# MarSaKi/VLN-BEVBert

Measured on AMD Instinct MI355X. Metric: pretrain_samples_per_sec, higher is better.
Workload: dtype bf16+fp32-residual

## Files before the change

include/bevbert_hip.h:

```cpp
#ifndef BEVBERT_HIP_H
#define BEVBERT_HIP_H

#include <stdint.h>

#ifdef __cplusplus
extern "C" {
#endif

typedef struct ihipStream_t* hipStream_t;

#define BEVBERT_F32 0
#define BEVBERT_BF16 1
#define BEVBERT_F16 2

const char* bevbert_last_error(void);
int bevbert_version(void);
int bevbert_hip_error_reset(void);
const char* bevbert_arch(void);
const char* bevbert_attn_last_path(int backward);
const char* bevbert_attn_plan(int B, int nh, int Lq, int Lk, int dtype, int impl, int has_key_mask, int has_bias,
                              float drop_p, int has_bits, int bits_ready, int want_dbias, int ncu, int backward);

int bevbert_bev_lift_bin(const float* depths, const float* T_c2w, const float* T_w2c, const float* S_w2c,
                         const float* pix_scale, int B, int V, int hw, float depth_scale, int dim, float res,
// ... 25 lines not shown
                                                float drop_p, uint64_t seed, uint64_t offset, hipStream_t stream);
int bevbert_layernorm_post_fwd(const void* x, const float* bias, const float* gamma, const float* beta,
                               const void* post1, const void* post2, void* y, void* z_out, float* mean, float* rstd,
                               int rows, int H, float eps, int dtype, hipStream_t stream);
int bevbert_layernorm_bwd(const void* dy, const void* z, const float* mean, const float* rstd, const float* gamma,
                          void* dz, void* dx, float* dgamma, float* dbeta, float* dbias, float* workspace, int rows,
                          int H, int dtype, float drop_p, uint64_t seed, uint64_t offset, int accumulate,
                          hipStream_t stream);
int bevbert_layernorm_bwd_add(const void* dy, const void* z, const float* mean, const float* rstd, const float* gamma,
                              void* dz, void* dx, const void* dz_add, float* dgamma, float* dbeta, float* dbias,
                              float* workspace, int rows, int H, int dtype, float drop_p, uint64_t seed, uint64_t offset,
                              int accumulate, hipStream_t stream);
int bevbert_layernorm_res32_fwd(const void* x, const float* bias, const void* residual, int residual_dtype,
                                const float* gamma, const float* beta, void* y16, float* y32, float* z32, float* mean,
                                float* rstd, int rows, int H, float eps, float drop_p, uint64_t seed, uint64_t offset,
                                hipStream_t stream);
int bevbert_layernorm_res32_chain_fwd(const void* x, const float* bias, const float* z_prev, const float* mean_prev,
                                      const float* rstd_prev, const float* gamma_prev, const float* beta_prev,
                                      const float* gamma, const float* beta, void* y16, float* y32, float* z32,
                                      float* mean, float* rstd, int rows, int H, float eps, float drop_p, uint64_t seed,
                                      uint64_t offset, hipStream_t stream);
int bevbert_layernorm_res32_bwd(const void* dy16, const float* dy32, const float* z32, const float* mean,
                                const float* rstd, const float* gamma, void* dz, void* dx16, float* dgamma,
                                float* dbeta, float* dbias, float* workspace, int rows, int H, float drop_p, uint64_t seed,
                                uint64_t offset, int accumulate, int dz_dtype,
                                hipStream_t stream);
int64_t bevbert_colsum_workspace_floats(int total_cols);
int bevbert_colsum_partial_rows(int rows);
int bevbert_colsum_finalize(const float* partials, int nblocks, int nwhich, int C, float* out0, float* out1,
                            float* out2, int accumulate, hipStream_t stream);
int bevbert_colsum_partials(const void* dy, float* partials, int rows, int C, int dtype, hipStream_t stream);
int bevbert_multi_finalize(const void* tasks, int ntasks, hipStream_t stream);
int bevbert_multi_accum(const void* tasks, int ntasks, hipStream_t stream);
int bevbert_set_fold_norm_slots(float* slots, int capacity);
int bevbert_sumsq_tasks(const void* tasks, int ntasks, hipStream_t stream);

int bevbert_embed_sum_layernorm_fwd(const int64_t* ids, const void* word, const void* pos, const void* type_row,
                                    const float* gamma, const float* beta, void* y, void* z_out, float* mean,
                                    float* rstd, int rows, int L, int H, float eps, int dtype, float drop_p,
                                    uint64_t seed, uint64_t offset, hipStream_t stream);

int bevbert_embedding_grad(const int64_t* ids, const void* d, float* table_grad, int rows, int H, int padding_idx,
                           int dtype, hipStream_t stream);

int64_t bevbert_smallk_workspace_floats(int rows, int K, int H);
int bevbert_smallk_linear_layernorm_fwd(const float* feat, const float* weight, const float* bias, const float* gamma,
                                        const float* beta, const void* post1, const void* table, const int64_t* idx,
                                        void* y, float* mean, float* rstd, int rows, int K, int H, float eps, int dtype,
                                        hipStream_t stream);
int bevbert_smallk_linear_layernorm_bwd(const void* dy, const float* feat, const float* weight, const float* bias,
                                        const float* mean, const float* rstd, const float* gamma, float* dweight,
                                        float* dbias, float* dgamma, float* dbeta, float* workspace, int rows, int K,
                                        int H, int dtype, hipStream_t stream);

int bevbert_colsum_any(const void* dy, float* out, int rows, int C, int dtype, int accumulate, hipStream_t stream);

int bevbert_weighted_mean_fwd(const float* x, const float* w, const float* denom_dev, float denom, int n, float* out,
                              hipStream_t stream);
int bevbert_weighted_mean_bwd(const float* dout, const float* w, const float* denom_dev, float denom, int n, float* dx,
                              hipStream_t stream);

int bevbert_sem_select(const uint8_t* mask1, const uint8_t* mask2, int n, int cap, int classes, int64_t* idx, float* valid,
                       float* denom, hipStream_t stream);
int bevbert_bce_rows_fwd(const void* logits, const uint8_t* labels, const int64_t* idx, float* out, int rows, int C, int dtype,
                         hipStream_t stream);
int bevbert_bce_rows_bwd(const void* logits, const uint8_t* labels, const int64_t* idx, const float* g, void* dlogits, int rows,
// ... 286 lines not shown
```

vln_bevbert_amd/arena.py:

```python
import math

import torch

from . import lib
from .lib import ptr, stream


def call(name, *args):
    from . import ops
    return ops.call(name, *args)

CHUNK = 1024
_ZERO_KERNEL = __import__("os").environ.get("BEVBERT_ZERO_KERNEL", "0") == "1"
NO_DECAY = ("bias", "LayerNorm.bias", "LayerNorm.weight")


def _round_up(n, m):
    return (n + m - 1) // m * m


class ParamArena:
    _serial = 0

    def __init__(self, module, device, compute_dtype=torch.float32, groups=()):
# ... 40 lines not shown
        self._flags_host = torch.zeros(off // CHUNK, dtype=torch.uint8)
        self._seg_of = {}
        for start, end, decay, seg in seg_meta:
            if decay:
                self._flags_host[start // CHUNK:end // CHUNK] |= 1
            for n in seg:
                self._seg_of[n] = (start // CHUNK, end // CHUNK)
        self.flags = self._flags_host.to(dev)
        self.chunk_steps = torch.zeros(off // CHUNK, dtype=torch.int32, device=dev)
        self._touched = set()
        self._flags_dirty = False
        self.publish_grads = True
        self.allreduce_group = None
        self.defer_allreduce = False
        self._cb_queued = False
        self._fresh = []
        self._published = []
        self._param_versions = None
        self.step_count = 0
        self._scalars = torch.zeros(4, dtype=torch.float32, device=dev)
        self._partials = torch.zeros(1024, dtype=torch.float32, device=dev)
        self.named = named
        for n, p in named:
            o, k = self.slices[n]
            view = self.params[o:o + k].view(p.shape)
            view.copy_(p.data.to(dev, torch.float32))
            p.data = view
            p.main_grad = self.grads[o:o + k].view(p.shape)
            p.compute = self.shadow[o:o + k].view(p.shape) if self.shadow is not None else p.data
            p.arena = self
            p.arena_name = n
        self._index = {n: i for i, (n, _) in enumerate(named)}
        self.fold_store = False
        ParamArena._serial += 1
        self.fold_key = ("arena", ParamArena._serial)
        tables = {id(m.weight) for m in module.modules() if isinstance(m, torch.nn.Embedding)}
        self._fold_ranges = []
        for o, k, _ in sorted((*self.slices[n], n) for n, p in named if p.dim() >= 2 and id(p) not in tables):
            if self._fold_ranges and self._fold_ranges[-1][1] == o:
                self._fold_ranges[-1][1] = o + k
            else:
                self._fold_ranges.append([o, o + k])
        self._fold_starts = [a for a, _ in self._fold_ranges]
        self._fold_comp = {}
        self.sync_shadow()
        self._param_versions = sum(p._version for _, p in named)

    def packed(self, names, shape):
        o0, _ = self.slices[names[0]]
        total = 0
        for n in names:
            o, k = self.slices[n]
            assert o == o0 + total, f"{names} are not contiguous in the arena"
            total += k
        assert total == math.prod(shape)
        src = self.shadow if self.shadow is not None else self.params
        return src[o0:o0 + total].view(shape), self.grads[o0:o0 + total].view(shape)

    def touch(self, param):
        n = param.arena_name
        if n not in self._touched:
            self._touched.add(n)
            a, b = self._seg_of[n]
            self._flags_host[a:b] |= 2
            self._flags_dirty = True
        if self.publish_grads:
# ... 48 lines not shown
        if v != self._param_versions:
            if self._param_versions is not None:
                self.sync_shadow()
            self._param_versions = v

    def sync_shadow(self):
        if self.shadow is not None:
            call("bevbert_cast_f32", ptr(self.params), ptr(self.shadow), self.numel, lib.dtype_code(self.compute_dtype),
                 stream())

    def sync(self):
        if self.device.type == "cuda":
            from . import ops
            ops.WgradStream.flush_all()
            cur = torch.cuda.current_stream(self.device)
            for side in ops.Branches.side_streams():
                if ops.Branches.enabled or side not in ops.WgradStream.streams or ops.WgradStream.dirty:
                    cur.wait_stream(side)
            ops.WgradStream.dirty = False
            ops.WgradStream.release()

    def store_ok(self, sink_ptr, n):
        import bisect
        off, rem = divmod(sink_ptr - self.grads.data_ptr(), 4)
        if rem or off < 0 or off + n > self.numel:
            return False
        i = bisect.bisect_right(self._fold_starts, off) - 1
        return i >= 0 and off + n <= self._fold_ranges[i][1]

    def _arm_fold(self):
        from . import ops
        ops.ReduceQueue.store_ok = self.store_ok if self.fold_store else None
        ops.ReduceQueue.fold_norm = None

    def _name_at(self, sink_ptr):
        off = (sink_ptr - self.grads.data_ptr()) // 4
        return next((n for n, (o, k) in self.slices.items() if o <= off < o + k), f"arena offset {off}")

    def fold_check_zero(self, stores):
        base = self.grads.data_ptr()
        views = [self.grads[(p - base) // 4:(p - base) // 4 + n] for p, n in stores]
        counts = torch.stack([torch.count_nonzero(v) for v in views]).tolist()
        bad = [(self._name_at(p), c) for (p, _), c in zip(stores, counts) if c]
        if bad:
            raise lib.BevBertHipError(
                "store-mode fold: the gradient of " + ", ".join(f"{n} ({c} non-zero elements)" for n, c in bad[:4])
                + " is not zero before the step's fold -- something other than the split-K fold writes it, or the arena "
                "was not zeroed for this step (BEVBERT_FOLD_STORE=0 turns the store mode off)")

    def _fold_complement(self, entry):
        ent = self._fold_comp.get(id(entry))
        if ent is not None and ent[0] is entry:
            return ent[1:]
        if torch.cuda.is_current_stream_capturing():
            raise lib.BevBertHipError("fold-norm complement table missing during graph capture (warm-up steps build it)")
        import numpy as np
        base, recs, pos = self.grads.data_ptr(), [], 0
        for p, n, _ in sorted(entry["norm_jobs"]) + [(base + 4 * self.numel, 0, 0)]:
            o = (p - base) // 4
            for a in range(pos, o, 16384):
                recs.append((base + 4 * a, (min(a + 16384, o) - a) // 4))
            pos = o + n
            assert pos % 4 == 0, "fold sinks are float4-aligned"
        from . import ops
        if entry["nslots"] + len(recs) > ops.ReduceQueue.SLOT_CAPACITY:
            return None
# ... 116 lines not shown
```

vln_bevbert_amd/csrc/optimizer.hip:

```cpp
#include <math.h>
#include <type_traits>

#include "rowops_common.h"

#define ACCUM_U 4
#define ACCUM_SC 4
template <typename T, bool STORE = false>
__device__ __forceinline__ float accum_fold(const T* part_, float* sink_, size_t stride4, size_t n4, int S, size_t first,
                                            size_t step) {
  const BB_GLOBAL T* __restrict__ part = (const BB_GLOBAL T*)part_;
  BB_GLOBAL float* __restrict__ sink = (BB_GLOBAL float*)sink_;
  float sq = 0.f;
  for (size_t i = first; i < n4; i += ACCUM_U * step) {
    size_t idx[ACCUM_U];
    float4 acc[ACCUM_U];
#pragma unroll
    for (int u = 0; u < ACCUM_U; ++u) {
      idx[u] = i + u * step < n4 ? i + u * step : n4 - 1;
      if constexpr (STORE) acc[u] = make_float4(0.f, 0.f, 0.f, 0.f);
      else acc[u] = gld4<float>(sink + idx[u] * 4);
    }
    int s = 0;
    for (; s + ACCUM_SC <= S; s += ACCUM_SC) {
      float4 v[ACCUM_SC][ACCUM_U];
// ... 29 lines not shown
                                                             int S, size_t n4) {
  accum_fold<T>(partials, sink, n4, n4, S, (size_t)blockIdx.x * 256 + threadIdx.x, (size_t)gridDim.x * 256);
}

struct AccumTask {
  const void* partials;
  float* sink;
  unsigned long long n4_total;
  unsigned int off4, n4;
  int S, dtype;
};
#define ACCUM_STORE 0x100
#define ACCUM_NORM 0x200
__device__ __forceinline__ float block_sum_256(float s) {
  __shared__ float sh[4];
  s = wave_sum(s);
  if ((threadIdx.x & 63) == 0) sh[threadIdx.x >> 6] = s;
  __syncthreads();
  return (sh[0] + sh[1]) + (sh[2] + sh[3]);
}
template <typename T, bool STORE>
__device__ __forceinline__ float accum_task(const AccumTask& t) {
  return accum_fold<T, STORE>((const T*)t.partials + (size_t)t.off4 * 4, t.sink, t.n4_total, t.n4, t.S, threadIdx.x, 256);
}
__global__ __launch_bounds__(256) void multi_accum_kernel(const AccumTask* __restrict__ tasks, float* __restrict__ slots,
                                                          unsigned int capacity) {
  const AccumTask t = tasks[blockIdx.x];
  const bool bf16 = (t.dtype & 0xff) == BB_BF16;
  float sq;
  if (t.dtype & ACCUM_STORE) sq = bf16 ? accum_task<bf16_raw, true>(t) : accum_task<float, true>(t);
  else sq = bf16 ? accum_task<bf16_raw, false>(t) : accum_task<float, false>(t);
  const unsigned int slot = (unsigned int)t.dtype >> 12;
  if ((t.dtype & ACCUM_NORM) && slot < capacity) {
    sq = block_sum_256(sq);
    if (threadIdx.x == 0) slots[slot] = sq;
  }
}

__global__ __launch_bounds__(256) void sumsq_kernel(const float* __restrict__ g, size_t n4, float* __restrict__ partials) {
  float s = 0.f;
  for (size_t i = (size_t)blockIdx.x * 256 + threadIdx.x; i < n4; i += (size_t)gridDim.x * 256) {
    const float4 v = *reinterpret_cast<const float4*>(g + i * 4);
    s += (v.x * v.x + v.y * v.y) + (v.z * v.z + v.w * v.w);
  }
  __shared__ float sh[4];
  s = wave_sum(s);
  if ((threadIdx.x & 63) == 0) sh[threadIdx.x >> 6] = s;
  __syncthreads();
  if (threadIdx.x == 0) partials[blockIdx.x] = (sh[0] + sh[1]) + (sh[2] + sh[3]);
}

struct SumsqTask {
  const float* ptr;
  unsigned int n4, slot;
};
__global__ __launch_bounds__(256) void sumsq_tasks_kernel(const SumsqTask* __restrict__ tasks, float* __restrict__ slots,
                                                          unsigned int capacity) {
  const SumsqTask t = tasks[blockIdx.x];
  if (t.slot >= capacity) return;
  const unsigned int n4 = t.n4 < 4096u ? t.n4 : 4096u;
  float s = 0.f;
  if (n4) {
    const BB_GLOBAL float* __restrict__ g = (const BB_GLOBAL float*)t.ptr;
    float4 v[16];
#pragma unroll
    for (int u = 0; u < 16; ++u) {
// ... 76 lines not shown
template <typename TO>
__global__ __launch_bounds__(256) void cast_f32_kernel(const float* __restrict__ src, TO* __restrict__ dst, size_t n4) {
  for (size_t i = (size_t)blockIdx.x * 256 + threadIdx.x; i < n4; i += (size_t)gridDim.x * 256)
    st4<TO>(dst + i * 4, *reinterpret_cast<const float4*>(src + i * 4));
}

BEVBERT_API int bevbert_accum_partials(const void* partials, float* sink, int S, int64_t n, int dtype,
                                       hipStream_t stream) {
  BB_REQUIRE(n % 4 == 0 && S >= 1, "accum_partials: n must be a multiple of 4 and S >= 1");
  if (n == 0) return BB_OK;
  size_t nb = ((size_t)n / 4 + 255) / 256;
  if (nb > 8192) nb = 8192;
  const bool type_ok = bb_with_type(dtype, [&](auto t) {
    using T = decltype(t);
    hipLaunchKernelGGL(accum_partials_kernel<T>, dim3(nb), dim3(256), 0, stream, (const T*)partials, sink, S, (size_t)n / 4);
  });
  if (!type_ok) return bb_dtype_unsupported("accum_partials", dtype);
  BB_CHECK_LAUNCH("accum_partials");
  return BB_OK;
}

BEVBERT_API int bevbert_multi_accum(const void* tasks, int ntasks, hipStream_t stream) {
  static_assert(sizeof(AccumTask) == 40, "AccumTask is part of the C ABI");
  if (ntasks <= 0) return BB_OK;
  BB_REQUIRE(tasks != nullptr, "multi_accum: null task table");
  int capacity = 0;
  float* slots = bb_fold_norm_slots(&capacity);
  hipLaunchKernelGGL(multi_accum_kernel, dim3(ntasks), dim3(256), 0, stream, (const AccumTask*)tasks, slots,
                     (unsigned int)(slots ? capacity : 0));
  BB_CHECK_LAUNCH("multi_accum");
  return BB_OK;
}

BEVBERT_API int bevbert_sumsq_tasks(const void* tasks, int ntasks, hipStream_t stream) {
  static_assert(sizeof(SumsqTask) == 16, "SumsqTask is part of the C ABI");
  if (ntasks <= 0) return BB_OK;
  int capacity = 0;
  float* slots = bb_fold_norm_slots(&capacity);
  BB_REQUIRE(tasks != nullptr && slots != nullptr, "sumsq_tasks: null task table, or no slot array registered");
  hipLaunchKernelGGL(sumsq_tasks_kernel, dim3(ntasks), dim3(256), 0, stream, (const SumsqTask*)tasks, slots,
                     (unsigned int)capacity);
  BB_CHECK_LAUNCH("sumsq_tasks");
  return BB_OK;
}

BEVBERT_API int bevbert_grad_norm_clip(const float* grads, int64_t n, float pre_scale, float max_norm,
                                       float* partials, float* scalars, hipStream_t stream) {
  BB_REQUIRE(n % 4 == 0, "grad_norm_clip: n must be a multiple of 4");
  hipLaunchKernelGGL(sumsq_kernel, dim3(1024), dim3(256), 0, stream, grads, (size_t)n / 4, partials);
  hipLaunchKernelGGL(clip_coef_kernel, dim3(1), dim3(256), 0, stream, partials, 1024, pre_scale, max_norm, scalars);
  BB_CHECK_LAUNCH("grad_norm_clip");
  return BB_OK;
}

BEVBERT_API int bevbert_clip_from_slots(const float* slots, int n, float pre_scale, float max_norm, float* scalars,
                                        hipStream_t stream) {
  BB_REQUIRE(n >= 0 && (slots != nullptr || n == 0) && scalars != nullptr, "clip_from_slots: null pointer or negative count");
  hipLaunchKernelGGL(clip_coef_kernel, dim3(1), dim3(256), 0, stream, slots, n, pre_scale, max_norm, scalars);
  BB_CHECK_LAUNCH("clip_from_slots");
  return BB_OK;
}

BEVBERT_API int bevbert_adamw_step(float* params, const float* grads, float* exp_avg, float* exp_avg_sq,
                                   void* params_bf16, const uint8_t* chunk_flags, int* chunk_steps, int64_t n,
                                   const float* grad_scale_dev, const float* lr_dev, float lr, float beta1,
                                   float beta2, float eps, float weight_decay, hipStream_t stream) {
// ... 27 lines not shown
```

vln_bevbert_amd/ops_gemm.py:

```python
import os as _os

import torch
import torch.nn.functional as F

from . import lib
from .lib import dtype_code, ptr, stream
from .ops_core import RT, _LT_WS_BYTES, _compute, _gemm, _mark_touched, _sink, call
from .ops_reduce import ReduceQueue, WgradStream, _on_launch_stream, _partial_rows


_LT_ENABLED = _os.environ.get("BEVBERT_LT_GEMM", "1") == "1"


_LT_AUTOTUNE = int(_os.environ.get("BEVBERT_LT_AUTOTUNE", "32"))


_LT_UNSUPPORTED = set()


_LT_PLAN_BUDGET = int(_os.environ.get("BEVBERT_LT_PLAN_BUDGET", "8192"))


_LT_PLANS = {}

# ... 143 lines not shown
    return _on_launch_stream(lambda: dy2.t().mm(x2))


_SPLITK_ENABLED = _os.environ.get("BEVBERT_SPLITK", "1") == "1"


_SPLITK_MAX = int(_os.environ.get("BEVBERT_SPLITK_MAX", "16"))


def _split_k(M, N, K):
    if not _SPLITK_ENABLED:
        return 1
    tiles = ((N + 255) // 256) * ((K + 255) // 256)
    s = 1
    while s * 2 <= min(_SPLITK_MAX, M // 640) and s * 2 * tiles <= 256 and M % (s * 2) == 0:
        s *= 2
    return s


def _wgrad_into(sink, dy2, x2):
    M, N = dy2.shape
    K = x2.shape[1]
    if dy2.dtype == torch.float32 and not (_LT_ENABLED and dy2.is_cuda):
        if dy2.is_cuda:
            _warn_fallback("wgrad", N, K, M, "BEVBERT_LT_GEMM=0")
        _gemm("wgrad", lambda: _on_launch_stream(lambda: sink.addmm_(dy2.t(), x2)), N, K, M)
        return None
    S = _split_k(M, N, K) if dy2.dtype != torch.float32 else 1
    if not (S > 1 and dy2.is_contiguous() and x2.is_contiguous()):
        S = 1
    batched = WgradStream.DEFER_FINALIZE and (N * K) % 4 == 0 and dy2.is_cuda
    part = _gemm("wgrad", lambda: _linear_wgrad(dy2, x2, S, scratch=batched), N, K, M)
    if batched:
        ReduceQueue.add_accum(part.data_ptr(), sink.data_ptr(), S, N * K, dtype_code(part))
        WgradStream._keep.append(part)
        return None
    if (N * K) % 4 == 0:
        call("bevbert_accum_partials", ptr(part), ptr(sink), S, N * K, dtype_code(part), stream())
    else:
        _on_launch_stream(lambda: sink.add_(part if S == 1 else part.sum(0)))
    return part


def _param_grads(w_sink, b_sink, dyc, xc):
    if w_sink is not None:
        part = _wgrad_into(w_sink, dyc, xc)
        if part is not None and lib._override is not None:
            WgradStream._keep.append(part)
    if b_sink is not None:
        C = dyc.shape[1]
        if WgradStream.DEFER_FINALIZE and dyc.shape[0] > 0:
            nb = _partial_rows(dyc.shape[0])
            part = RT.scratch.alloc(nb * C * 4, dyc.device)
            call("bevbert_colsum_partials", ptr(dyc), part, dyc.shape[0], C, dtype_code(dyc), stream())
            ReduceQueue.add(part, nb, 1, C, (ptr(b_sink), None, None))
        else:
            ws = RT.workspace(dyc.device, lib.load().bevbert_colsum_workspace_floats(C))
            call("bevbert_colsum", ptr(dyc), ptr(b_sink), ptr(ws), dyc.shape[0], C, dtype_code(dyc), 1, stream())


class _Linear(torch.autograd.Function):

    @staticmethod
    def forward(ctx, x, weight, bias, w_c, b_c, tap=False):
        y = _gemm("fwd", lambda: _linear_fwd(x, w_c, b_c), x.numel() // x.shape[-1], w_c.shape[0], w_c.shape[1])
        ctx.save_for_backward(x, w_c)
        ctx.params = (weight, bias)
# ... 190 lines not shown
```

vln_bevbert_amd/ops_reduce.py:

```python
import math
import os as _os

import torch

from . import lib
from .lib import stream
from .ops_core import Branches, RT, call


class WgradStream:

    enabled = _os.environ.get("BEVBERT_WGRAD_STREAM", "1") == "1"
    BATCH = int(_os.environ.get("BEVBERT_WGRAD_BATCH", "6"))
    DEFER_FINALIZE = _os.environ.get("BEVBERT_DEFER_FINALIZE", "1") == "1"
    OWN_STREAM = _os.environ.get("BEVBERT_WGRAD_OWN_STREAM", "1") == "1"
    stream = None
    streams = []
    NSTREAMS = int(_os.environ.get("BEVBERT_WGRAD_STREAMS", "2"))
    _rr = 0
    _target = None
    dirty = False
    _keep = []
    _pending = {}
    _events = []
# ... 23 lines not shown
        if not fns:
            return
        if cls.stream is None:
            shared = Branches._streams.get(producer.device.index) if Branches.enabled and not cls.OWN_STREAM else None
            from .hwqueues import side_stream
            cls.stream = shared if shared is not None else side_stream(producer.device)
            Branches._streams["wgrad"] = cls.stream
            cls._events = [torch.cuda.Event() for _ in range(64)]
            cls.streams = [cls.stream]
            for i in range(1, cls.NSTREAMS):
                st = side_stream(producer.device)
                Branches._streams[f"wgrad{i}"] = st
                cls.streams.append(st)
        if final or len(cls.streams) == 1:
            target = cls.stream
        else:
            cls._rr += 1
            target = cls.streams[cls._rr % len(cls.streams)]
        if producer.cuda_stream != target.cuda_stream:
            ev = cls._events[cls._next_event % len(cls._events)]
            cls._next_event += 1
            ev.record(producer)
            target.wait_event(ev)
        if final:
            for st in cls.streams[1:]:
                target.wait_stream(st)
            ReduceQueue.wait_producers(target)
        lib.set_stream_override(target.cuda_stream)
        cls._target = target
        cls.dirty = True
        try:
            for fn in fns:
                fn()
        finally:
            lib.set_stream_override(None)
            cls._target = None
            fns.clear()

    @classmethod
    def flush_all(cls):
        if ReduceQueue.jobs or ReduceQueue.accum_jobs:
            dev = torch.device("cuda", torch.cuda.current_device())
            if cls.active(dev):
                h = lib.stream()
                slot = cls._pending.get(h)
                if slot is None:
                    slot = cls._pending[h] = (torch.cuda.current_stream(dev), [])
                slot[1].append(lambda: ReduceQueue.flush(dev))
                mine = slot
                for other in cls._pending.values():
                    if other is not mine:
                        cls._flush(other)
                cls._flush(mine, final=True)
                return
            ReduceQueue.wait_producers(torch.cuda.current_stream(dev))
            ReduceQueue.flush(dev)
        for slot in cls._pending.values():
            cls._flush(slot)

    @classmethod
    def release(cls):
        cls._keep.clear()

    @classmethod
    def drop_pending(cls):
        for _, fns in cls._pending.values():
            fns.clear()
        cls._keep.clear()


class ScratchRing:

    INITIAL = 256 << 20

# ... 3 lines not shown
        self.size = 0
        self.buf = None
        self.base = 0
        self.off = 0
        self.ci = 0
        self._chunks = []
        self._old = []

    def reset(self):
        self.off = self.ci = 0
        if self._chunks:
            self.buf, self.base, self.size = self._chunks[0]

    def total_bytes(self):
        return sum(c[2] for c in self._chunks)

    def alloc(self, nbytes, device):
        n = (int(nbytes) + 255) & ~255
        if n > self.nbytes:
            raise lib.BevBertHipError(f"scratch ring: {n} bytes requested, buffer size {self.nbytes} (BEVBERT_SCRATCH_MB)")
        if self.off + n > self.size:
            if self.ci == 0 and self.size < self.nbytes:
                if torch.device(device).type == "cuda" and torch.cuda.is_current_stream_capturing():
                    raise lib.BevBertHipError("scratch ring would have to grow during graph capture: run one more "
                                              "eager step first, or start larger (BEVBERT_SCRATCH_INITIAL_MB)")
                new = min(self.nbytes, max(2 * self.size, self.off + n, self.INITIAL))
                if self.buf is not None:
                    self._old.append(self.buf)
                self.buf = torch.empty(new, dtype=torch.uint8, device=device)
                self.base, self.size, self.off = self.buf.data_ptr(), new, 0
                self._chunks[:1] = [[self.buf, self.base, self.size]]
            elif self.ci + 1 < len(self._chunks):
                self._enter(self.ci + 1)
            elif not (ReduceQueue.jobs or ReduceQueue.accum_jobs):
                self._enter(0)
            else:
                if torch.device(device).type == "cuda" and torch.cuda.is_current_stream_capturing():
                    raise lib.BevBertHipError("scratch ring would need another buffer during graph capture: run one more "
                                              "eager step first, or raise BEVBERT_SCRATCH_MB")
                if self.total_bytes() + self.nbytes > self.max_total:
                    raise lib.BevBertHipError(
                        f"one backward pass queued more than {self.total_bytes() >> 20} MB of partial sums for its column "
                        "reductions: raise BEVBERT_SCRATCH_MAX_MB if that is intended")
                buf = torch.empty(self.nbytes, dtype=torch.uint8, device=device)
                self._chunks.append([buf, buf.data_ptr(), self.nbytes])
                self._enter(len(self._chunks) - 1)
        p = self.base + self.off
        self.off += n
        return p

    def _enter(self, ci):
        self.ci, self.off = ci, 0
        self.buf, self.base, self.size = self._chunks[ci]

    def tensor(self, shape, dtype, device):
        nbytes = math.prod(shape) * torch.empty((), dtype=dtype).element_size()
        p = self.alloc(nbytes, device)
        o = p - self.base
        return self.buf[o:o + nbytes].view(dtype).view(shape)


SCRATCH = ScratchRing(int(_os.environ.get("BEVBERT_SCRATCH_MB", "6144")) << 20,
                      int(_os.environ.get("BEVBERT_SCRATCH_MAX_MB", "65536")) << 20)


ScratchRing.INITIAL = int(_os.environ.get("BEVBERT_SCRATCH_INITIAL_MB", "256")) << 20
RT.scratch = SCRATCH


class ReduceQueue:

    jobs = []
    accum_jobs = []
    table_bytes = {}
    producers = {}
    _tables = {}
    _accum_tables = {}
    _dtype = None
    _adtype = None
    FOLD_STORE = _os.environ.get("BEVBERT_FOLD_STORE", "1") == "1"
    STORE, NORM = 0x100, 0x200
    SLOT_CAPACITY = 1 << 16
    store_ok = None
    fold_norm = None
    _slots = None

    @classmethod
    def slots(cls, device):
        if cls._slots is None:
            if torch.cuda.is_current_stream_capturing():
                raise lib.BevBertHipError("fold-norm slot array missing during graph capture (warm-up steps allocate it)")
            cls._slots = torch.zeros(cls.SLOT_CAPACITY, dtype=torch.float32, device=device)
        return cls._slots

    @classmethod
    def register_slots(cls, device):
        s = cls.slots(device)
        lib.load().bevbert_set_fold_norm_slots(s.data_ptr(), s.numel())
        return s

    @classmethod
    def _note_producer(cls):
        st = WgradStream._target
        if st is None:
            if not torch.cuda.is_available():
                return
            st = torch.cuda.current_stream()
        cls.producers[st.cuda_stream] = st

    @classmethod
    def wait_producers(cls, consumer):
        for h, st in cls.producers.items():
            if h != consumer.cuda_stream:
                consumer.wait_stream(st)
        cls.producers = {}

    @classmethod
    def drop_pending(cls):
        cls.jobs, cls.accum_jobs, cls.producers = [], [], {}

    @classmethod
    def add_accum(cls, partials_ptr, sink_ptr, S, n, dtype):
        cls.accum_jobs.append((partials_ptr, sink_ptr, S, n, dtype))
        cls._note_producer()

    @classmethod
    def _build_accum(cls, jobs, device, flags=None, slot0=0):
        import numpy as np
        if cls._adtype is None:
            cls._adtype = np.dtype([("partials", "<u8"), ("sink", "<u8"), ("n4_total", "<u8"), ("off4", "<u4"),
                                    ("n4", "<u4"), ("S", "<i4"), ("dtype", "<i4")])
        parts, slot = [], slot0
        flags = flags if flags is not None else [0] * len(jobs)
        for (partials_ptr, sink_ptr, S, n, dt), fl in zip(jobs, flags):
            n4 = n // 4
            off = np.arange(0, n4, 4096, dtype=np.int64)
            t = np.zeros(len(off), dtype=cls._adtype)
            t["partials"] = partials_ptr
            t["sink"] = sink_ptr + off * 16
            t["n4_total"] = n4
            t["off4"] = off
            t["n4"] = np.minimum(4096, n4 - off)
            t["S"] = S
            word = np.full(len(off), dt | (fl & (cls.STORE | cls.NORM)), dtype=np.int64)
            if fl & cls.NORM:
                word |= (slot + np.arange(len(off), dtype=np.int64)) << 12
                slot += len(off)
            t["dtype"] = word.astype(np.uint32).view(np.int32)
            parts.append(t)
        table = np.concatenate(parts) if parts else np.zeros(0, dtype=cls._adtype)
        dev = torch.from_numpy(table.view(np.uint8).copy()).to(device)
        cls.table_bytes[dev.data_ptr()] = int(sum(S * n * (4 if dt == lib.F32 else 2) + (4 * n if fl & cls.STORE else 8 * n)
                                                  for (_, _, S, n, dt), fl in zip(jobs, flags)))
        return dev, len(table)

    @classmethod
    def _plan_fold(cls, jobs, ok):
        rounds, seen, last = [[]], [set()], {}
        for job in jobs:
            r = 0
            while job[1] in seen[r]:
                r += 1
                if r == len(rounds):
                    rounds.append([])
                    seen.append(set())
            rounds[r].append(job)
            seen[r].add(job[1])
# ... 18 lines not shown
        cls.jobs.append((partials_ptr, nblocks, nwhich, C, outs[0] or 0, outs[1] or 0, outs[2] or 0, accumulate))
        cls._note_producer()

    @classmethod
    def _build(cls, jobs, device):
        import numpy as np
        if cls._dtype is None:
            cls._dtype = np.dtype([("partials", "<u8"), ("out", "<u8"), ("nblocks", "<i4"), ("row_stride", "<i4"),
                                   ("col0", "<i4"), ("ncols", "<i4"), ("accumulate", "<i4"), ("pad", "<i4")])
        parts = []
        for partials_ptr, nblocks, nwhich, C, o0, o1, o2, acc in jobs:
            ntile = (C + 63) // 64
            tiles = np.arange(ntile, dtype=np.int64)
            for which, out in enumerate((o0, o1, o2)[:nwhich]):
                if not out:
                    continue
                t = np.zeros(ntile, dtype=cls._dtype)
                t["partials"] = partials_ptr
                t["out"] = out + tiles * 256
                t["nblocks"] = nblocks
                t["row_stride"] = nwhich * C
                t["col0"] = which * C + tiles * 64
                t["ncols"] = np.minimum(64, C - tiles * 64)
                t["accumulate"] = acc
                parts.append(t)
        table = np.concatenate(parts) if parts else np.zeros(0, dtype=cls._dtype)
        dev = torch.from_numpy(table.view(np.uint8).copy()).to(device)
        cls.table_bytes[dev.data_ptr()] = int(4 * (table["nblocks"].astype(np.int64) * table["ncols"]).sum()
                                              + 4 * (table["ncols"] * (1 + (table["accumulate"] != 0))).sum()) if len(table) else 0
        return dev, len(table)

    @classmethod
    def flush(cls, device):
        if cls.accum_jobs:
            jobs = tuple(cls.accum_jobs)
            cls.accum_jobs = []
            ok, cls.store_ok, cls.fold_norm = (cls.store_ok if cls.FOLD_STORE else None), None, None
            owner = getattr(ok, "__self__", ok)
            akey = (jobs, None if ok is None else getattr(owner, "fold_key", id(owner)))
            aent = cls._accum_tables.get(akey)
            if aent is None:
                if torch.cuda.is_current_stream_capturing():
                    raise lib.BevBertHipError("accumulate task table missing during graph capture (warm-up steps build it)")
                if len(cls._accum_tables) > 256:
                    cls._accum_tables.clear()
                rounds, flags = cls._plan_fold(jobs, ok)
                tasks_of = lambda j: (j[3] // 4 + 4095) // 4096
                n_norm = sum(tasks_of(j) for rnd, fl in zip(rounds, flags) for j, f in zip(rnd, fl) if f & cls.NORM)
                if n_norm > cls.SLOT_CAPACITY // 2:
                    flags = [[f & ~cls.NORM for f in fl] for fl in flags]
                tables, nslots, norm_jobs = [], 0, []
                for rnd, fl in zip(rounds, flags):
                    tables.append(cls._build_accum(tuple(rnd), device, fl, nslots))
                    for j, f in zip(rnd, fl):
                        if f & cls.NORM:
                            norm_jobs.append((j[1], j[3], nslots))
                            nslots += tasks_of(j)
                aent = {
                    "tables": tables, "nslots": nslots, "norm_jobs": norm_jobs, "fresh": True,
                    "flagged": any(f for fl in flags for f in fl),
                    "stores": [(j[1], j[3]) for rnd, fl in zip(rounds, flags) for j, f in zip(rnd, fl) if f & cls.STORE]}
                if aent["stores"] and hasattr(owner, "fold_check_zero"):
                    _on_launch_stream(lambda: owner.fold_check_zero(aent["stores"]))
                cls._accum_tables[akey] = aent
            if aent["flagged"]:
                cls.register_slots(device)
            for table, n in aent["tables"]:
                call("bevbert_multi_accum", table.data_ptr(), n, stream())
            if aent["nslots"]:
                cls.fold_norm = {"owner": owner, "entry": aent}
        if not cls.jobs:
            return
        key = tuple(cls.jobs)
        cls.jobs = []
        ent = cls._tables.get(key)
        if ent is None:
            if torch.cuda.is_current_stream_capturing():
                raise lib.BevBertHipError("reduction task table missing during graph capture (warm-up steps build it)")
            if len(cls._tables) > 256:
                cls._tables.clear()
            rounds, seen = [[]], [set()]
            for job in key:
                outs = {o for o in job[4:7] if o}
                r = 0
                while outs & seen[r]:
                    r += 1
                    if r == len(rounds):
                        rounds.append([])
                        seen.append(set())
                rounds[r].append(job)
                seen[r] |= outs
            ent = cls._tables[key] = [cls._build(tuple(r), device) for r in rounds]
        for table, n in ent:
            call("bevbert_multi_finalize", table.data_ptr(), n, stream())


def _on_launch_stream(fn):
# ... 15 lines not shown
```

vln_bevbert_amd/train.py:

```python
import contextlib
import os
import random

import torch
import torch.distributed as dist

from . import capture, ops
from .static_step import GraphedStep, StaticBatch


def warmup_linear_lr(step, base_lr, warmup_steps, total_steps):
    f = step / warmup_steps if step < warmup_steps else max(0, (total_steps - step) / (total_steps - warmup_steps))
    lr = base_lr * f
    return lr if lr > 0 else 1e-8


def load_gemm_tuning():
    import os
    path = os.path.join(os.path.dirname(os.path.abspath(__file__)), "tunableop_results.csv")
    if os.environ.get("BEVBERT_GEMM_TUNING", "1") != "1" or not os.path.exists(path):
        return 0
    try:
        import torch.cuda.tunable as tunable
        tunable.enable(True)
# ... 319 lines not shown

    def _hook_text(self, module, inputs, output):
        if output.requires_grad and torch.is_grad_enabled():
            output.register_hook(lambda g: (self.reducer.phase_a(), g)[1])
        return output

    def broadcast_state(self, src=0):
        if not (dist.is_available() and dist.is_initialized()):
            return
        a = self.arena
        dist.broadcast(a.params, src=src, group=self.reducer.group)
        if a.exp_avg is not None:
            dist.broadcast(a.exp_avg, src=src, group=self.reducer.group)
            dist.broadcast(a.exp_avg_sq, src=src, group=self.reducer.group)
            dist.broadcast(a.chunk_steps, src=src, group=self.reducer.group)
        for b in self.model.buffers():
            dist.broadcast(b, src=src, group=self.reducer.group)
        a.sync_shadow()

    def _step_seed(self):
        return (self.seed + self.rank) * 1000003 + self.global_step

    def forward_backward(self, task, batch):
        self.global_step += 1
        ops.RT.new_step(self._step_seed(), plan_key=self._plan_key(task, batch))
        return self._forward_backward(task, batch)

    @staticmethod
    def _plan_key(task, batch):
        return (task, batch.signature) if isinstance(batch, StaticBatch) else None

    def _forward_backward(self, task, batch):
        self._reset_map_hooks()
        self.arena.zero_grad(overlap=self.overlap_zero)
        try:
            if isinstance(batch, StaticBatch):
                loss = self.model.loss_mean(batch.tensors, task)
            else:
                loss = self.model(batch, task, compute_loss=True).mean()
        finally:
            self.arena.wait_zero()
        if self.reducer is not None and self.reducer.timeline is not None:
            self.backward_start = torch.cuda.Event(enable_timing=True)
            self.backward_start.record()
        if loss.is_cuda and loss.dim() == 0:
            one = self.__dict__.get("_one")
            if one is None or one.dtype != loss.dtype or one.device != loss.device:
                one = self._one = torch.ones((), dtype=loss.dtype, device=loss.device)
            loss.backward(gradient=one)
        else:
            loss.backward()
        self.arena.sync()
        self.reducer.finish()
        return loss.detach()

    def optimizer_step(self, lr=None, fused_norm=False):
        if lr is None:
            lr = warmup_linear_lr(self.global_step, self.lr, self.warmup, self.total)
        self.arena.clip_and_step(lr, self.betas, 1e-6, self.wd, self.grad_norm, grad_pre_scale=1.0 / self.world,
                                 fused_norm=fused_norm)

    def step(self, task, batch):
        if isinstance(batch, StaticBatch) and self.use_graphs and self.capture_ok and batch.capturable and ops.RT.trace is None:
            return self._static_step(task, batch)
        loss = self.forward_backward(task, batch)
        self.optimizer_step(fused_norm=True)
# ... 114 lines not shown
```

Baseline: 3789.

## Fold split-K weight-gradient partials early, right after each wgrad GEMM

Adds an early-fold path. Weight gradients whose sink is written exactly once per step (learned from a warm-up step's plan keyed by arena and task) have their split-K partials reduced into the gradient arena, with norm contributions recorded, immediately after the GEMM. This replaces deferring all of them to one batched accumulate at flush time. The aim is to overlap the reduction with remaining backward work and shrink the tail accumulate before the optimizer. It adds plan bookkeeping, invalidation when a step deviates, a new fold_weight kernel, and extra small launches per GEMM batch.

```diff
diff --git a/include/bevbert_hip.h b/include/bevbert_hip.h
--- a/include/bevbert_hip.h
+++ b/include/bevbert_hip.h
@@ -81,6 +81,8 @@
 int bevbert_colsum_partials(const void* dy, float* partials, int rows, int C, int dtype, hipStream_t stream);
 int bevbert_multi_finalize(const void* tasks, int ntasks, hipStream_t stream);
 int bevbert_multi_accum(const void* tasks, int ntasks, hipStream_t stream);
+int bevbert_fold_weight(const void* partials, float* sink, int S, int64_t n, int dtype_and_flags, int slot0,
+                        hipStream_t stream);
 int bevbert_set_fold_norm_slots(float* slots, int capacity);
 int bevbert_sumsq_tasks(const void* tasks, int ntasks, hipStream_t stream);
 
diff --git a/vln_bevbert_amd/arena.py b/vln_bevbert_amd/arena.py
--- a/vln_bevbert_amd/arena.py
+++ b/vln_bevbert_amd/arena.py
@@ -96,6 +96,7 @@
             p.arena_name = n
         self._index = {n: i for i, (n, _) in enumerate(named)}
         self.fold_store = False
+        self.fold_task = None
         ParamArena._serial += 1
         self.fold_key = ("arena", ParamArena._serial)
         tables = {id(m.weight) for m in module.modules() if isinstance(m, torch.nn.Embedding)}
@@ -210,6 +211,8 @@
         from . import ops
         ops.ReduceQueue.store_ok = self.store_ok if self.fold_store else None
         ops.ReduceQueue.fold_norm = None
+        task, self.fold_task = self.fold_task, None
+        ops.ReduceQueue.early_key = (self.fold_key, task) if self.fold_store and task is not None else None
 
     def _name_at(self, sink_ptr):
         off = (sink_ptr - self.grads.data_ptr()) // 4
diff --git a/vln_bevbert_amd/csrc/optimizer.hip b/vln_bevbert_amd/csrc/optimizer.hip
--- a/vln_bevbert_amd/csrc/optimizer.hip
+++ b/vln_bevbert_amd/csrc/optimizer.hip
@@ -85,6 +85,26 @@
   else sq = bf16 ? accum_task<bf16_raw, false>(t) : accum_task<float, false>(t);
   const unsigned int slot = (unsigned int)t.dtype >> 12;
   if ((t.dtype & ACCUM_NORM) && slot < capacity) {
+    sq = block_sum_256(sq);
+    if (threadIdx.x == 0) slots[slot] = sq;
+  }
+}
+
+template <typename T, bool STORE>
+__global__ __launch_bounds__(256) void fold_weight_kernel(const T* __restrict__ partials, float* __restrict__ sink, size_t n4,
+                                                          int S, int norm, unsigned int slot0, float* __restrict__ slots,
+                                                          unsigned int capacity) {
+  const size_t off4 = (size_t)blockIdx.x * 4096;
+  AccumTask t;
+  t.partials = partials;
+  t.sink = sink + off4 * 4;
+  t.n4_total = n4;
+  t.off4 = (unsigned int)off4;
+  t.n4 = (unsigned int)(n4 - off4 < 4096 ? n4 - off4 : 4096);
+  t.S = S;
+  float sq = accum_task<T, STORE>(t);
+  const unsigned int slot = slot0 + blockIdx.x;
+  if (norm && slot < capacity) {
     sq = block_sum_256(sq);
     if (threadIdx.x == 0) slots[slot] = sq;
   }
@@ -227,6 +247,31 @@
   return BB_OK;
 }
 
+BEVBERT_API int bevbert_fold_weight(const void* partials, float* sink, int S, int64_t n, int dtype_and_flags, int slot0,
+                                    hipStream_t stream) {
+  BB_REQUIRE(n >= 0 && n % 4 == 0 && S >= 1 && slot0 >= 0, "fold_weight: n must be a multiple of 4, S >= 1, slot0 >= 0");
+  BB_REQUIRE((dtype_and_flags & ~(0xff | ACCUM_STORE | ACCUM_NORM)) == 0, "fold_weight: unknown flag bits");
+  if (n == 0) return BB_OK;
+  BB_REQUIRE(partials != nullptr && sink != nullptr, "fold_weight: null pointer");
+  const size_t n4 = (size_t)n / 4;
+  BB_REQUIRE(n4 <= 0xffffffffull, "fold_weight: more than 2^32 float4 groups in one weight");
+  int capacity = 0;
+  float* slots = bb_fold_norm_slots(&capacity);
+  const int norm = (dtype_and_flags & ACCUM_NORM) != 0;
+  const bool store = (dtype_and_flags & ACCUM_STORE) != 0;
+  const dim3 grid((unsigned int)((n4 + 4095) / 4096));
+  const bool type_ok = bb_with_type(dtype_and_flags & 0xff, [&](auto t) {
+    using T = decltype(t);
+    bb_with_bool(store, [&](auto st) {
+      hipLaunchKernelGGL((fold_weight_kernel<T, decltype(st)::value>), grid, dim3(256), 0, stream, (const T*)partials, sink,
+                         n4, S, norm, (unsigned int)slot0, slots, (unsigned int)(slots ? capacity : 0));
+    });
+  });
+  if (!type_ok) return bb_dtype_unsupported("fold_weight", dtype_and_flags & 0xff);
+  BB_CHECK_LAUNCH("fold_weight");
+  return BB_OK;
+}
+
 BEVBERT_API int bevbert_sumsq_tasks(const void* tasks, int ntasks, hipStream_t stream) {
   static_assert(sizeof(SumsqTask) == 16, "SumsqTask is part of the C ABI");
   if (ntasks <= 0) return BB_OK;
diff --git a/vln_bevbert_amd/ops_gemm.py b/vln_bevbert_amd/ops_gemm.py
--- a/vln_bevbert_amd/ops_gemm.py
+++ b/vln_bevbert_amd/ops_gemm.py
@@ -199,7 +199,8 @@
     batched = WgradStream.DEFER_FINALIZE and (N * K) % 4 == 0 and dy2.is_cuda
     part = _gemm("wgrad", lambda: _linear_wgrad(dy2, x2, S, scratch=batched), N, K, M)
     if batched:
-        ReduceQueue.add_accum(part.data_ptr(), sink.data_ptr(), S, N * K, dtype_code(part))
+        if not ReduceQueue.fold_early(part.data_ptr(), sink.data_ptr(), S, N * K, dtype_code(part), sink.device):
+            ReduceQueue.add_accum(part.data_ptr(), sink.data_ptr(), S, N * K, dtype_code(part))
         WgradStream._keep.append(part)
         return None
     if (N * K) % 4 == 0:
diff --git a/vln_bevbert_amd/ops_reduce.py b/vln_bevbert_amd/ops_reduce.py
--- a/vln_bevbert_amd/ops_reduce.py
+++ b/vln_bevbert_amd/ops_reduce.py
@@ -79,6 +79,7 @@
         try:
             for fn in fns:
                 fn()
+            ReduceQueue.issue_early_batch(producer.device)
         finally:
             lib.set_stream_override(None)
             cls._target = None
@@ -86,7 +87,8 @@
 
     @classmethod
     def flush_all(cls):
-        if ReduceQueue.jobs or ReduceQueue.accum_jobs:
+        if (ReduceQueue.jobs or ReduceQueue.accum_jobs or ReduceQueue.early_done
+                or any(fns for _, fns in cls._pending.values())):
             dev = torch.device("cuda", torch.cuda.current_device())
             if cls.active(dev):
                 h = lib.stream()
@@ -156,7 +158,7 @@
                 self._chunks[:1] = [[self.buf, self.base, self.size]]
             elif self.ci + 1 < len(self._chunks):
                 self._enter(self.ci + 1)
-            elif not (ReduceQueue.jobs or ReduceQueue.accum_jobs):
+            elif not (ReduceQueue.jobs or ReduceQueue.accum_jobs or ReduceQueue.early_done):
                 self._enter(0)
             else:
                 if torch.device(device).type == "cuda" and torch.cuda.is_current_stream_capturing():
@@ -208,6 +210,14 @@
     store_ok = None
     fold_norm = None
     _slots = None
+    FOLD_EARLY = _os.environ.get("BEVBERT_FOLD_EARLY", "1") != "0"
+    EARLY_PER_GEMM = _os.environ.get("BEVBERT_FOLD_EARLY", "1") == "gemm"
+    _early_batch = []
+    _early_tables = {}
+    early_key = None
+    early_done = {}
+    _early_plans = {}
+    _early_broken = False
 
     @classmethod
     def slots(cls, device):
@@ -242,6 +252,7 @@
     @classmethod
     def drop_pending(cls):
         cls.jobs, cls.accum_jobs, cls.producers = [], [], {}
+        cls.early_done, cls._early_broken, cls._early_batch = {}, False, []
 
     @classmethod
     def add_accum(cls, partials_ptr, sink_ptr, S, n, dtype):
@@ -249,14 +260,70 @@
         cls._note_producer()
 
     @classmethod
-    def _build_accum(cls, jobs, device, flags=None, slot0=0):
+    def fold_early(cls, partials_ptr, sink_ptr, S, n, dtype, device):
+        ok = cls.store_ok
+        if ok is None or cls.early_key is None or not (cls.FOLD_EARLY and cls.FOLD_STORE):
+            return False
+        plan = cls._early_plans.get(cls.early_key)
+        if plan is None or plan["n"].get(sink_ptr) != n:
+            return False
+        if sink_ptr in cls.early_done:
+            cls._early_broken = True
+            return False
+        if not cls.early_done:
+            cls.register_slots(device)
+            if plan["fresh"] and not torch.cuda.is_current_stream_capturing():
+                plan["fresh"] = False
+                owner = getattr(ok, "__self__", ok)
+                if hasattr(owner, "fold_check_zero"):
+                    _on_launch_stream(lambda: owner.fold_check_zero(list(plan["n"].items())))
+        cls._early_batch.append((partials_ptr, sink_ptr, S, n, dtype, plan["slot0"][sink_ptr]))
+        cls.early_done[sink_ptr] = n
+        cls._note_producer()
+        if cls.EARLY_PER_GEMM or WgradStream._target is None:
+            cls.issue_early_batch(device)
+        return True
+
+    @classmethod
+    def issue_early_batch(cls, device):
+        jobs, cls._early_batch = tuple(cls._early_batch), []
+        if not jobs:
+            return
+        flags = cls.STORE | cls.NORM
+        if len(jobs) == 1:
+            part, sink, S, n, dt, slot0 = jobs[0]
+            call("bevbert_fold_weight", part, sink, S, n, dt | flags, slot0, stream())
+            return
+        ent = cls._early_tables.get(jobs)
+        if ent is None:
+            if torch.cuda.is_current_stream_capturing():
+                raise lib.BevBertHipError("early-fold task table missing during graph capture (warm-up steps build it)")
+            if len(cls._early_tables) > 1024:
+                WgradStream._keep.extend(t for t, _ in cls._early_tables.values())
+                cls._early_tables.clear()
+            ent = cls._early_tables[jobs] = cls._build_accum(tuple(j[:5] for j in jobs), device, [flags] * len(jobs),
+                                                             slots=[j[5] for j in jobs])
+        call("bevbert_multi_accum", ent[0].data_ptr(), ent[1], stream())
+
+    @classmethod
+    def plan_early(cls, single):
+        slot0, pos = {}, 0
+        for p, n in single:
+            slot0[p] = pos
+            pos += (n // 4 + 4095) // 4096
+        return {"slot0": slot0, "n": dict(single), "nslots": pos, "fresh": True}
+
+    @classmethod
+    def _build_accum(cls, jobs, device, flags=None, slot0=0, slots=None):
         import numpy as np
         if cls._adtype is None:
             cls._adtype = np.dtype([("partials", "<u8"), ("sink", "<u8"), ("n4_total", "<u8"), ("off4", "<u4"),
                                     ("n4", "<u4"), ("S", "<i4"), ("dtype", "<i4")])
         parts, slot = [], slot0
         flags = flags if flags is not None else [0] * len(jobs)
-        for (partials_ptr, sink_ptr, S, n, dt), fl in zip(jobs, flags):
+        for i, ((partials_ptr, sink_ptr, S, n, dt), fl) in enumerate(zip(jobs, flags)):
+            if slots is not None:
+                slot = slots[i]
             n4 = n // 4
             off = np.arange(0, n4, 4096, dtype=np.int64)
             t = np.zeros(len(off), dtype=cls._adtype)
@@ -341,12 +408,25 @@
 
     @classmethod
     def flush(cls, device):
-        if cls.accum_jobs:
+        cls.issue_early_batch(device)
+        if cls.accum_jobs or cls.early_done:
             jobs = tuple(cls.accum_jobs)
             cls.accum_jobs = []
             ok, cls.store_ok, cls.fold_norm = (cls.store_ok if cls.FOLD_STORE else None), None, None
             owner = getattr(ok, "__self__", ok)
-            akey = (jobs, None if ok is None else getattr(owner, "fold_key", id(owner)))
+            early, broken, cls.early_done, cls._early_broken = cls.early_done, cls._early_broken, {}, False
+            learn = ok is not None and cls.FOLD_EARLY and cls.early_key is not None
+            plan = cls._early_plans.get(cls.early_key) if learn else None
+            stale = (plan is not None or bool(early)) and (plan is None or broken or early.keys() != plan["n"].keys())
+            if stale:
+                if torch.cuda.is_current_stream_capturing():
+                    raise lib.BevBertHipError("a captured step did not follow the early-fold plan of its warm-up steps")
+                cls._early_plans.pop(cls.early_key, None)
+                plan, learn = None, False
+            if early and ok is not None:
+                ok = (lambda inner: lambda p, k: p not in early and inner(p, k))(ok)
+            akey = (jobs, None if ok is None else getattr(owner, "fold_key", id(owner)),
+                    tuple(early) if stale else plan and id(plan))
             aent = cls._accum_tables.get(akey)
             if aent is None:
                 if torch.cuda.is_current_stream_capturing():
@@ -356,22 +436,31 @@
                 rounds, flags = cls._plan_fold(jobs, ok)
                 tasks_of = lambda j: (j[3] // 4 + 4095) // 4096
                 n_norm = sum(tasks_of(j) for rnd, fl in zip(rounds, flags) for j, f in zip(rnd, fl) if f & cls.NORM)
-                if n_norm > cls.SLOT_CAPACITY // 2:
+                if n_norm + (plan["nslots"] if plan else 0) > cls.SLOT_CAPACITY // 2:
                     flags = [[f & ~cls.NORM for f in fl] for fl in flags]
                 tables, nslots, norm_jobs = [], 0, []
+                if plan is not None:
+                    nslots, norm_jobs = plan["nslots"], [(p, n, plan["slot0"][p]) for p, n in plan["n"].items()]
                 for rnd, fl in zip(rounds, flags):
-                    tables.append(cls._build_accum(tuple(rnd), device, fl, nslots))
+                    if rnd:
+                        tables.append(cls._build_accum(tuple(rnd), device, fl, nslots))
                     for j, f in zip(rnd, fl):
                         if f & cls.NORM:
                             norm_jobs.append((j[1], j[3], nslots))
                             nslots += tasks_of(j)
                 aent = {
-                    "tables": tables, "nslots": nslots, "norm_jobs": norm_jobs, "fresh": True,
+                    "tables": tables, "nslots": 0 if stale else nslots, "norm_jobs": norm_jobs, "fresh": True,
+                    "plan": plan,
+                    "single": [(j[1], j[3]) for j, f in zip(rounds[0], flags[0]) if f == cls.STORE | cls.NORM],
                     "flagged": any(f for fl in flags for f in fl),
                     "stores": [(j[1], j[3]) for rnd, fl in zip(rounds, flags) for j, f in zip(rnd, fl) if f & cls.STORE]}
                 if aent["stores"] and hasattr(owner, "fold_check_zero"):
                     _on_launch_stream(lambda: owner.fold_check_zero(aent["stores"]))
                 cls._accum_tables[akey] = aent
+            if learn and plan is None and aent["single"]:
+                if len(cls._early_plans) > 256:
+                    cls._early_plans.clear()
+                cls._early_plans[cls.early_key] = cls.plan_early(aent["single"])
             if aent["flagged"]:
                 cls.register_slots(device)
             for table, n in aent["tables"]:
diff --git a/vln_bevbert_amd/train.py b/vln_bevbert_amd/train.py
--- a/vln_bevbert_amd/train.py
+++ b/vln_bevbert_amd/train.py
@@ -375,6 +375,7 @@
 
     def _forward_backward(self, task, batch):
         self._reset_map_hooks()
+        self.arena.fold_task = (task, batch.signature if isinstance(batch, StaticBatch) else None)
         self.arena.zero_grad(overlap=self.overlap_zero)
         try:
             if isinstance(batch, StaticBatch):
```

Result: no change. 3813 (median of 6 runs) (+0.6%).
